# awslabs/crowd-coachable-recommendations

Hardware: AMD Instinct MI355X
Metric: queries/sec, exhaustive inner-product top-100 retrieval (NQ-shaped 2,681,468 x 768 bf16 corpus) (higher is better)
Workload: dtype bf16

## Files before the change

### crowd-coachable-recommendations_amd/ccrec_amd/_lib.py

```python
import ctypes
import os

_HERE = os.path.dirname(os.path.abspath(__file__))
LIB_PATH = os.path.join(os.path.dirname(_HERE), "lib", "libccr_hip.so")

CCR_OK = 0
CCR_ERR_INVALID, CCR_ERR_HIP, CCR_ERR_WORKSPACE, CCR_ERR_BLOCK_ID = -1, -2, -3, -4
DTYPE_F32, DTYPE_F16, DTYPE_BF16 = 0, 1, 2
SEARCH_DEFAULT, SEARCH_FORCE_DENSE, SEARCH_FORCE_FUSED, SEARCH_ASYNC = 0, 1, 2, 4
SCORES_CANONICAL, SCORES_MFMA = 0, 1

EXPORTS = [
    "ccr_last_error", "ccr_version", "ccr_pack_bf16", "ccr_pack_bf16_ex", "ccr_meanpool_pack_bf16", "ccr_meanpool_pack_bf16_ex", "ccr_index_create",
    "ccr_index_create_with_norms", "ccr_index_destroy",
    "ccr_index_rows", "ccr_index_dim", "ccr_search_workspace_bytes", "ccr_search", "ccr_search_last_stats",
    "ccr_merge_topk", "ccr_merge_topk_strided", "ccr_apply_block", "ccr_inbatch_ce_workspace_bytes", "ccr_inbatch_ce_fwd", "ccr_inbatch_ce_bwd", "ccr_inbatch_ce_bwd_dev", "ccr_rank_metrics",
    "ccr_search_finish", "ccr_scores", "ccr_search_blocked_workspace_bytes", "ccr_search_blocked",
    "ccr_search_sparse_prior_workspace_bytes", "ccr_search_sparse_prior", "ccr_colsum_bf16", "ccr_meanpool_bwd", "ccr_bm25_index_create", "ccr_bm25_index_destroy", "ccr_bm25_search_workspace_bytes",
    "ccr_bm25_search", "ccr_pack_bf16_padded", "ccr_shard_message_bytes", "ccr_search_shard", "ccr_shard_message_fill", "ccr_merge_shard_messages",
    "ccr_attention_bf16", "ccr_add_layernorm", "ccr_meanpool_pack_bf16_packed", "ccr_embed_layernorm", "ccr_gelu_bf16",
    "ccr_attention_half", "ccr_add_layernorm_half", "ccr_embed_layernorm_half", "ccr_gelu_half", "ccr_merge_short_lists",
    "ccr_bm25_search_workspace_bytes_k", "ccr_bm25_search_last_stats", "ccr_bm25_index_set_idf", "ccr_inbatch_pack3_bf16", "ccr_inbatch_ce_fwd_f32",
    "ccr_search_stream_wait_main_pass", "ccr_pool_ce_workspace_bytes", "ccr_pool_ce_fwd", "ccr_pool_ce_fwd_f32", "ccr_pool_ce_bwd_dev",
    "ccr_bpr_sample", "ccr_bpr_frozen_workspace_bytes", "ccr_bpr_frozen_fwd", "ccr_bpr_frozen_bwd_dev",
# ... 14 lines not shown
QSPLIT_VERSION = 105
THR_PHASES_VERSION = 106
OPTIM_VERSION = 107
ENCODER_PACKED_TRAIN_VERSION = 108
HALF_INDEX_VERSION = 109
AMP_OPTIM_VERSION = 110

SHARD_HEADER_BYTES = 32
SHARD_MAGIC = 0x4D524343


class ShardHeader(ctypes.Structure):
    _fields_ = [("magic", ctypes.c_uint32), ("n_flagged", ctypes.c_uint32), ("k_valid", ctypes.c_uint32),
                ("n_covered", ctypes.c_uint32), ("row_offset", ctypes.c_int64), ("n_rows", ctypes.c_int64)]


class SearchStats(ctypes.Structure):
    _fields_ = [("path", ctypes.c_int32), ("n_fallback", ctypes.c_int32), ("sample_tiles", ctypes.c_int32),
                ("ranges", ctypes.c_int32), ("cap", ctypes.c_int32), ("sublists", ctypes.c_int32),
                ("n_candidates", ctypes.c_int64), ("ms_sample", ctypes.c_float), ("ms_threshold", ctypes.c_float),
                ("ms_main", ctypes.c_float), ("ms_select", ctypes.c_float), ("ms_fallback", ctypes.c_float),
                ("ms_total", ctypes.c_float), ("n_retried", ctypes.c_int32), ("n_dense", ctypes.c_int32),
                ("main_launches", ctypes.c_int32), ("opt_rank", ctypes.c_int32), ("main_tile_queries", ctypes.c_int32),
                ("skipped_tiles", ctypes.c_int32)]


class AdamwSegment(ctypes.Structure):
    _fields_ = [("param", ctypes.c_void_p), ("grad", ctypes.c_void_p), ("exp_avg", ctypes.c_void_p), ("exp_avg_sq", ctypes.c_void_p),
                ("shadow", ctypes.c_void_p), ("n", ctypes.c_int64), ("decay", ctypes.c_float), ("step_size", ctypes.c_float),
                ("bc2_sqrt", ctypes.c_float), ("shadow_dtype", ctypes.c_int32)]


class AdamwControl(ctypes.Structure):
    _fields_ = [("coef", ctypes.c_float), ("skip", ctypes.c_int32), ("norm", ctypes.c_float), ("scale", ctypes.c_float),
                ("growth_tracker", ctypes.c_int32), ("skipped_total", ctypes.c_int32), ("reserved", ctypes.c_uint32 * 10)]


CONTROL_WORDS = {name: i for i, (name, _) in enumerate(AdamwControl._fields_[:6])}


class CcrError(RuntimeError):
    pass


_lib = None


# ... 140 lines not shown
```

### crowd-coachable-recommendations_amd/csrc/ccr_api.hip

```cpp
#include <stdarg.h>
#include <stdlib.h>
#include <string.h>

#include <math.h>

#include <algorithm>
#include <mutex>
#include <set>
#include <utility>
#include <vector>

#include "ccr_index.h"
#include "ccr_narrow.h"
#include "ccr_topk_device.h"

namespace ccr {

static thread_local char g_err[512] = "";
void set_error(const char *fmt, ...) {
    va_list ap;
    va_start(ap, fmt);
    vsnprintf(g_err, sizeof(g_err), fmt, ap);
    va_end(ap);
}
// ... 403 lines not shown
    return CCR_OK;
}


static int fused_stats(ccr_index *ix, uint32_t nflag, unsigned long long ncand) {
    const Plan &p = ix->plan;
    ccr_search_stats &st = ix->stats;
    float a = 0, b = 0;
    CCR_HIP_CHECK(hipEventElapsedTime(&st.ms_sample, ix->ev[EV_SAMPLE_BEGIN], ix->ev[EV_SAMPLE_END]));
    CCR_HIP_CHECK(hipEventElapsedTime(&a, ix->ev[EV_BEGIN], ix->ev[EV_SAMPLE_BEGIN]));
    CCR_HIP_CHECK(hipEventElapsedTime(&b, ix->ev[EV_SAMPLE_END], ix->ev[EV_MAIN_BEGIN]));
    st.ms_threshold = a + b;
    CCR_HIP_CHECK(hipEventElapsedTime(&st.ms_main, ix->ev[EV_MAIN_BEGIN], ix->ev[EV_MAIN_END]));
    CCR_HIP_CHECK(hipEventElapsedTime(&st.ms_select, ix->ev[EV_MAIN_END], ix->ev[EV_SELECT_END]));
    CCR_HIP_CHECK(hipEventElapsedTime(&st.ms_total, ix->ev[EV_BEGIN], ix->ev[EV_SELECT_END]));
    st.path = 1;
    st.n_fallback = (int32_t)nflag;
    st.sample_tiles = p.sample_tiles;
    st.ranges = p.narrow ? 1 : p.ranges;
    st.cap = p.narrow ? p.first_lay.cap[0] : p.cap;
    st.sublists = p.narrow ? p.first_sp : p.sublists;
    st.main_launches = 1 + (p.item_a ? 1 : 0) + (p.item_b ? 1 : 0);
    st.opt_rank = p.opt_rank;
    st.skipped_tiles = p.skip_sampled ? p.sample_tiles : 0;
    st.main_tile_queries = p.narrow ? 0 : p.tile_q;
    st.n_candidates = (int64_t)ncand;
    return CCR_OK;
}

static int recover_thresholds(const ccr_index *ix, const SearchWs &w, int nflag) {
    hipStream_t s = ix->pending.stream;
    ThresholdArgs t = threshold_args(ix, w);
    t.thr = w.thr_safe, t.cq = w.cq_safe;
    const int rc = launch_threshold(t, s);
    if (rc != CCR_OK) return rc;
    return launch_underfilled_to_retry(w.flag_list, 0, nflag, w.thr_safe, w.thr, s);
}

static int to_dense(const SearchWs &w, const uint32_t *list, int n, int &n_dense, hipStream_t s) {
    CCR_HIP_CHECK(hipMemcpyAsync(w.dense_list + n_dense, list, (size_t)n * 4, hipMemcpyDeviceToDevice, s));
    n_dense += n;
    return CCR_OK;
}

static int retry_group(ccr_index *ix, const SearchWs &w, const uint32_t *cur, int n_cur, int &n_dense) {
    const Plan &p = ix->plan;
// ... 189 lines not shown
        ix->have_events = true;
    }
    CCR_HIP_CHECK(hipEventRecord(ix->ev[EV_BEGIN], s));
    if (!p.fused) return search_dense(ix, w, Q_bf16, n_q, k, out_scores, out_ids, flags, s);
    ix->pending = {false, Q_bf16, n_q, k, out_scores, out_ids, (char *)workspace, s};

    CCR_HIP_CHECK(hipMemsetAsync(w.flag_count, 0, 64, s));
    if ((int64_t)p.ranges > p.tiles - (p.skip_sampled ? p.sample_tiles : 0)) CCR_HIP_CHECK(hipMemsetAsync(w.cnt, 0, (size_t)p.ranges * p.nq_pad * p.sublists * 4, s));
    int rc = launch_row_norms(Q_bf16, ix->dtype, n_q, ix->dim, w.qnorm, nullptr, nullptr, s);
    if (rc != CCR_OK) return rc;

    GemmArgs gs = gemm_args(ix, Q_bf16, n_q, p.nq_pad);
    gs.qgroups = p.qgroups;
    gs.n_vt = p.sample_tiles;
    gs.tile_stride = p.sample_stride;
    gs.ranges = p.sample_ranges;
    gs.gmax = w.gmax;
    CCR_HIP_CHECK(hipEventRecord(ix->ev[EV_SAMPLE_BEGIN], s));
    rc = launch_gemm(gs, ix->dtype, MAIN_32X32, EPI_GMAX, p.grid, s);
    if (rc != CCR_OK) return rc;
    CCR_HIP_CHECK(hipEventRecord(ix->ev[EV_SAMPLE_END], s));
    const bool skip_list = p.skip_sampled && ix->knobs.skip_list;
    ThresholdArgs t = threshold_args(ix, w);
    if (p.opt_rank) t.k = p.opt_rank;
    if (p.narrow) t.zero_cnt = w.cnt, t.zero_per_query = NARROW_SUBLISTS;
    if (skip_list) t.glist = w.glist, t.list_cap = skip_list_cap(p.opt_rank);
    rc = launch_threshold(t, s, &ix->thr_phases_used);
    if (rc != CCR_OK) return rc;

    CCR_HIP_CHECK(hipEventRecord(ix->ev[EV_MAIN_BEGIN], s));
    rc = p.narrow ? run_narrow_pass(ix, p, w, Q_bf16, n_q, s) : run_main_pass(ix, p, w, Q_bf16, n_q, s);
    if (rc != CCR_OK) return rc;
    CCR_HIP_CHECK(hipEventRecord(ix->ev[EV_MAIN_END], s));
    ix->main_pass_recorded = true;
    SelectArgs sel = select_args(ix, w);
    sel.ranges = p.first_nsub, sel.sp = p.first_sp, sel.lay = p.first_lay;
    sel.flag_count = w.flag_count, sel.flag_list = w.flag_list, sel.stat_cand = w.stat_cand;
    if (p.skip_sampled)
        sel.gmax = w.gmax, sel.sample_tiles = p.sample_tiles, sel.sample_stride = (int)p.sample_stride, sel.gmax_pitch = p.nq_pad;
    if (skip_list) sel.glist = w.glist, sel.list_cap = t.list_cap;
    rc = launch_select_rescore(sel, s);
    if (rc != CCR_OK) return rc;
    CCR_HIP_CHECK(hipEventRecord(ix->ev[EV_SELECT_END], s));

    if (!async) return search_complete(ix);
    if (flagged_out) CCR_HIP_CHECK(hipMemcpyAsync(flagged_out, w.flag_count, 4, hipMemcpyDeviceToDevice, s));
    CCR_HIP_CHECK(hipMemcpyAsync((void *)ix->host_flags, w.flag_count, 16, hipMemcpyDeviceToHost, s));
// ... 50 lines not shown
```

### crowd-coachable-recommendations_amd/csrc/ccr_index.h

```cpp
#pragma once
#include "ccr_common.h"
#include "ccr_plan.h"

namespace ccr {

enum MainKernel { MAIN_32X32, MAIN_16X16, MAIN_WIDE };
int launch_gemm(const GemmArgs &a, int dt, MainKernel kind, int epi, int grid, hipStream_t s);
int launch_shard_header(const ccr_shard_header &h, void *message, hipStream_t s);
int ensure_dynamic_lds(const void *kernel, size_t lds);
int launch_row_norms(const uint16_t *X, int dt, int64_t rows, int dim, float *norms, uint32_t *max_bits, uint32_t *tile_bits,
                     hipStream_t s);
int launch_tile_norms(const float *row_bounds, int64_t rows, uint32_t *tile_bits, uint32_t *max_bits, hipStream_t s);

struct ThresholdArgs {
    const float *gmax;
    int64_t n_groups, sample_stride;
    int n_q, nq_pad, dim;
    int k;
    const float *qnorm, *tile_norm;
    const uint32_t *dmax_bits;
    float *thr, *cq;
    uint32_t *zero_cnt = nullptr; int zero_per_query = 0;
    uint32_t *glist = nullptr; int list_cap = 0;
    int phases = 0;
};
int launch_threshold(const ThresholdArgs &a, hipStream_t s, int *phases_used = nullptr);

struct ThresholdUpdateArgs {
    const uint2 *cand;
    const uint32_t *cnt;
    CandLayout lay;
    int sp;
    int n_q, nq_pad, k, nsub;
    const float *cq, *tile_norm;
    float *thr;
    int nsub_part = 0, part_blocks = 0, prev_nsub = 0, prev_part = 0, prev_blocks = 0;
    int qb_per = 1;
    uint32_t *top = nullptr;
    bool top_in = false, top_out = false;
    int tile_q = TILE_Q;
};
// ... 83 lines not shown
```

### crowd-coachable-recommendations_amd/csrc/ccr_plan.h

```cpp
#pragma once
#include "ccr_common.h"
#include "ccr_narrow.h"

namespace ccr {

struct Knobs {
    int qgroups;
    int progressive;
    int max_phases;
    int mfma16;
    int sample_div;
    int ranges;
    int optimistic;
    int opt_rank;
    int max_lists;
    int narrow;
    int narrow_grid;
    int skip_sampled;
    int skip_list;
    int qsplit;
    int wide;
    int thr_phases;
    int narrow_groups;
};
struct KnobDef {
    const char *env;
    int Knobs::*field;
    int dflt;
};
inline constexpr KnobDef KNOB_DEFS[] = {
    {"CCR_QGROUPS", &Knobs::qgroups, 0},           {"CCR_PROGRESSIVE", &Knobs::progressive, 1},   {"CCR_PHASES", &Knobs::max_phases, 3},
    {"CCR_MFMA16", &Knobs::mfma16, -1},            {"CCR_SAMPLE_DIV", &Knobs::sample_div, 0},     {"CCR_RANGES", &Knobs::ranges, 0},
    {"CCR_OPTIMISTIC", &Knobs::optimistic, -1},    {"CCR_OPT_RANK", &Knobs::opt_rank, 0},         {"CCR_MAX_LISTS", &Knobs::max_lists, 0},
    {"CCR_NARROW", &Knobs::narrow, -1},            {"CCR_NARROW_GRID", &Knobs::narrow_grid, 0},   {"CCR_SKIP_SAMPLED", &Knobs::skip_sampled, -1},
    {"CCR_SKIP_LIST", &Knobs::skip_list, 1},       {"CCR_QSPLIT", &Knobs::qsplit, -1},            {"CCR_WIDE", &Knobs::wide, -1},
    {"CCR_THR_PHASES", &Knobs::thr_phases, 0},     {"CCR_NARROW_GROUPS", &Knobs::narrow_groups, NARROW_MAX_GROUPS},
};
static_assert(sizeof(KNOB_DEFS) / sizeof(KNOB_DEFS[0]) * sizeof(int) == sizeof(Knobs), "a row for every knob");
inline Knobs default_knobs() {
    Knobs kn;
    for (const KnobDef &d : KNOB_DEFS) kn.*d.field = d.dflt;
    return kn;
}
Knobs read_knobs();

struct Plan {
    int fused;
    int nq_pad;
    int qblocks;
    int tile_q;
    int main_qblocks;
    int main_qgroups;
    int main_qsplit;
    int64_t tiles;
    int64_t full_tiles;
    int sample_tiles;
    int64_t sample_stride;
    int sample_ranges;
    int ranges;
    int item_a;
    int item_b;
    int opt_rank;
    int skip_sampled;
    int qgroups;
    int cap;
    CandLayout cand;
    int grid;
    int rescore_cap;
    int rescore_regular;
    int select_compact;
    int mfma16;
    int sublists;
    int narrow;
    int narrow_groups;
    int first_nsub;
    int first_sp;
    CandLayout first_lay;
    int64_t cand_recs;
    size_t total;
    int64_t dense_rows_per_chunk;
};

constexpr int FALLBACK_ROWS = 16;

Plan make_plan(int64_t n_rows, int dim, int n_q, int k, int flags, int num_cu, const Knobs &kn);

inline int64_t round_up(int64_t v, int64_t m) { return (v + m - 1) / m * m; }
int pick_qgroups(int qblocks, int dim, const Knobs &kn, int tile_q = TILE_Q);
CandLayout one_segment(int cap);

struct Bump {
    size_t off;
    size_t take(size_t bytes) { const size_t o = off; off = (off + bytes + 255) / 256 * 256; return o; }
};

struct SearchWs {
    float *qnorm, *thr, *cq, *gmax;
    uint32_t *cnt;
    uint2 *cand;
    uint32_t *flag_count, *flag_list;
    unsigned long long *stat_cand;
    uint32_t *top;
    float *thr_safe, *cq_safe, *dense;
    uint32_t *glist;
// ... 10 lines not shown
```

### crowd-coachable-recommendations_amd/csrc/ccr_plan.hip

```cpp
#include <stdlib.h>
#include <string.h>

#include <math.h>

#include <algorithm>
#include <vector>

#include "ccr_index.h"
#include "ccr_topk_device.h"

namespace ccr {

Knobs read_knobs() {
    Knobs kn = default_knobs();
    for (const KnobDef &d : KNOB_DEFS)
        if (const char *e = getenv(d.env)) kn.*d.field = atoi(e);
    return kn;
}

constexpr double L2_RESIDENT_BYTES = 3.2 * 1048576.0, L2_MOSTLY_BYTES = 5.5 * 1048576.0;
constexpr double WIDE_TILE_COST = 1.37;
constexpr double MODEL_QUERIES = 3584.0;

static double tile_cost(const Plan &p) { return p.tile_q == WIDE_Q ? WIDE_TILE_COST : 1.0; }
static double query_scale(const Plan &p) { return (double)p.nq_pad / MODEL_QUERIES; }

static double gamma_upper(double r) { return 1.25 * (r + 4.75 * sqrt(r) + 8.0) / r; }

static double estimated_pass(int rank, double fs, int k) { return std::max((double)rank / fs, (double)k); }
static double sample_fraction(const Plan &p) { return 1.0 / ((double)p.tiles / (double)p.sample_tiles); }
static double estimated_pass_upper(const Plan &p, int k) {
    return gamma_upper((double)p.opt_rank) * estimated_pass(p.opt_rank, sample_fraction(p), k);
}
static double conservative_pass(const Plan &p, int k) { return (double)k * ((double)p.tiles / (double)p.sample_tiles) * 1.3 + 64.0; }

int pick_qgroups(int qblocks, int dim, const Knobs &kn, int tile_q) {
    {
        const int v = kn.qgroups;
        if ((v == 1 || v == 2 || v == 4 || v == 8) && qblocks % v == 0) return v;
    }
    const size_t block_bytes = (size_t)tile_q * dim * 2;
    int best = 1;
    for (int gq = 1; gq <= NUM_XCD; gq *= 2) {
        if (qblocks % gq) continue;
        best = gq;
        if ((size_t)(qblocks / gq) * block_bytes <= (size_t)3 << 20) break;
    }
    return best;
}

static int footprint_class(double bytes) { return bytes <= L2_RESIDENT_BYTES ? 0 : (bytes <= L2_MOSTLY_BYTES ? 1 : 2); }

static int pick_qsplit(int qblocks, int equal_groups, int dim, int tile_q, const Knobs &kn) {
    if (kn.qsplit == 0) return 0;
    const int v = kn.qgroups;
// ... 32 lines not shown
        }
    }
    return best_r;
}

constexpr size_t DENSE_SCRATCH_TARGET = (size_t)1 << 30;

struct MainPassChoice {
    int64_t sample, ranges;
    int item_a, item_b;
    int opt_rank;
    int skip;
};

static bool may_skip_sampled(const Plan &p, int64_t sample, const Knobs &kn) {
    if (kn.skip_sampled == 0 || p.narrow || sample < 1) return false;
    const int64_t stride = std::max<int64_t>(1, p.full_tiles / sample);
    return stride >= 2 && (sample - 1) * stride < p.full_tiles && sample < p.tiles;
}

static int optimistic_rank(int k, int64_t sample, int64_t tiles, const Knobs &kn, bool skip = false) {
    if (kn.opt_rank > 0) return kn.opt_rank;
    const double need = (double)k * (double)sample / (double)(skip ? tiles - sample : tiles);
    int r = 40;
    for (; r < 1 << 20; ++r) {
        const double a = 1.0 / (9.0 * r), t = 1.0 - a - 5.2 * sqrt(a);
        if (t > 0.0 && (double)r * t * t * t >= need) break;
    }
    return r;
}

static void range_window(const Plan &p, const Knobs &kn, int64_t &r_hi, int64_t &target) {
    int64_t max_lists = p.rescore_cap > 512 ? 2048 : 1024;
    if ((max_lists / p.sublists) * p.main_qblocks < p.grid) max_lists = 2048;
    if (kn.max_lists >= 64 && kn.max_lists < max_lists) max_lists = kn.max_lists;
    r_hi = std::min<int64_t>(max_lists / p.sublists, round_up(std::max<int64_t>(1, p.tiles / 8), NUM_XCD));
    target = std::min<int64_t>(r_hi, round_up(std::max<int64_t>(NUM_XCD, (int64_t)p.grid * 6 / p.main_qblocks), NUM_XCD));
}

static double sample_cost(const Plan &p, int64_t smp) {
    return (double)((smp * p.qblocks + p.grid - 1) / p.grid) + 0.015 * (double)smp * std::max(1.0, query_scale(p));
}

struct Best {
    double cost;
    MainPassChoice choice;
    void offer(double c, const MainPassChoice &ch) {
        if (c < cost) cost = c, choice = ch;
    }
};

static void price_range_count(const Plan &p, int k, const Knobs &kn, int64_t smp, int64_t R, int64_t target, bool reprice_skipped, Best &best) {
    const int nrc = NUM_XCD / p.main_qgroups, qb_per = p.main_qblocks / p.main_qgroups, per_x = p.grid / NUM_XCD;
    const double qscale = query_scale(p);
    const double select_per_range = 0.1 * qscale, hit_w = 0.014 * qscale, phase_w = 3.0;
    const double fs = (double)smp / (double)p.tiles;
    auto survivors = [&](double fa, double fb) -> double {
        if (fa <= 0.0) return (double)k / fs;
        if (fb <= 0.0) return (double)k * (fa / fs + (1.0 - fa) / fa);
        return (double)k * (fa / fs + fb / fa + (1.0 - fa - fb) / (fa + fb));
    };
    const int64_t items = R / nrc * qb_per;
    const double item_cost = ((double)((p.tiles + R - 1) / R) + 0.15) * tile_cost(p);
    auto rounds = [&](int64_t n) { return (double)((n + per_x - 1) / per_x); };
    const double common = sample_cost(p, smp) + select_per_range * (double)R + 1e-3 * std::abs((double)(R - target));
    const double single = rounds(items) * item_cost + hit_w * survivors(0.0, 0.0) + common;
    if (kn.optimistic != 1 && !reprice_skipped) best.offer(single, {smp, R, 0, 0, 0, 0});
    if (kn.optimistic != 0 && smp * GROUPS_PER_TILE >= 4 * 40) {
        const bool skip = reprice_skipped && may_skip_sampled(p, smp, kn);
        const int rank = optimistic_rank(k, smp, p.tiles, kn, skip);
        if ((int64_t)rank * 4 <= smp * GROUPS_PER_TILE) {
            const double opt_item = skip ? ((double)((p.tiles - smp + R - 1) / R) + 0.15) * tile_cost(p) : item_cost;
            const double opt = rounds(items) * opt_item + hit_w * estimated_pass(rank, fs, k) + common - (kn.optimistic == 1 ? 1e9 : 0.0);
            best.offer(opt, {smp, R, 0, 0, rank, skip ? 1 : 0});
        }
    }
    if (reprice_skipped || kn.progressive == 0 || p.narrow || !(items > per_x && (double)p.tiles / (double)R >= 8.0)) return;
    const double fa = (double)per_x / (double)items;
    best.offer((1.0 + rounds(items - per_x)) * item_cost + phase_w + hit_w * survivors(fa, 0.0) + common, {smp, R, per_x, 0, 0, 0});
    if (kn.max_phases < 3) return;
    for (int ph = 1; ph <= 3; ++ph) {
        const int64_t ib = (int64_t)per_x * (1 + ph);
        if (ib >= items) break;
        const double fb = (double)ph * per_x / (double)items;
        best.offer((1.0 + ph + rounds(items - ib)) * item_cost + 2.0 * phase_w + hit_w * survivors(fa, fb) + common, {smp, R, per_x, (int)ib, 0, 0});
    }
}

static MainPassChoice choose_main_pass(const Plan &p, int k, const std::vector<int64_t> &samples, const Knobs &kn, bool reprice_skipped = false) {
    int64_t r_hi, target;
    range_window(p, kn, r_hi, target);
// ... 72 lines not shown
    p.narrow = narrow ? nqt : 0;
    p.narrow_groups = narrow ? ngroups : 1;
}

static void choose_tile(const Search &s, Plan &p) {
    const Knobs &kn = s.kn;
    const int n_q = s.n_q, dim = s.dim;
    if (!p.narrow && p.mfma16 && dim % 32 == 0 && kn.wide != 0) {
        static const double per_flop_of_class[3] = {0.95, 0.97, 1.04};
        const int wb = (n_q + WIDE_Q - 1) / WIDE_Q;
        const double per_xcd = (double)(wb / pick_qgroups(wb, dim, kn, WIDE_Q)) * WIDE_Q * dim * 2.0;
        const double per_flop = per_flop_of_class[footprint_class(per_xcd)];
        if (kn.wide == 1 || (double)wb * WIDE_Q * per_flop < (double)p.qblocks * TILE_Q) {
            p.tile_q = WIDE_Q;
            p.main_qblocks = wb;
            p.nq_pad = (int)round_up(std::max<int64_t>(n_q, (int64_t)wb * WIDE_Q), TILE_Q);
            p.qblocks = p.nq_pad / TILE_Q;
            p.qgroups = pick_qgroups(p.qblocks, dim, kn);
        }
    }
    p.main_qgroups = pick_qgroups(p.main_qblocks, dim, kn, p.tile_q);
}

static void choose_launches(const Search &s, Plan &p, const std::vector<int64_t> &samples) {
    const Knobs &kn = s.kn;
    MainPassChoice choice = choose_main_pass(p, s.k, samples, kn);
    if (choice.opt_rank > 0 && may_skip_sampled(p, choice.sample, kn)) {
        const MainPassChoice skipped = choose_main_pass(p, s.k, {choice.sample}, kn, true);
        if (skipped.skip) choice = skipped;
    }
    p.sample_tiles = (int)choice.sample;
    p.sample_stride = std::max<int64_t>(1, p.full_tiles / choice.sample);
    p.sample_ranges = best_sample_ranges(choice.sample, p.qblocks, p.qgroups, p.grid);
    p.ranges = (int)choice.ranges;
    p.item_a = choice.item_a;
    p.item_b = choice.item_b;
    p.opt_rank = choice.opt_rank;
    p.skip_sampled = (p.opt_rank > 0 && !p.narrow) ? choice.skip : 0;
    p.main_qsplit = (!p.narrow && p.item_a == 0 && p.item_b == 0) ? pick_qsplit(p.main_qblocks, p.main_qgroups, s.dim, p.tile_q, kn) : 0;
}

static void price_skip_sampled(const Search &s, Plan &p) {
    if (!p.skip_sampled) return;
    const int k = s.k;
    const double join_rows = 256.0 * (double)p.sample_tiles * (1.0 - pow(1.0 - std::min(1.0, (double)k / (double)s.n_rows), 16.0));
    const double need = (double)k + (double)(k / 4) + 1.5 * join_rows + TILE_DOCS + 16;
    const double saved = 0.5 * (double)p.sample_tiles * p.main_qblocks * tile_cost(p) / (double)p.grid;
    const bool pays = 0.065 * join_rows * query_scale(p) < saved;
    if (need > 8192.0 || (s.kn.skip_sampled < 0 && !pays))
        p.skip_sampled = 0;
    else
        p.rescore_cap = std::min(8192, std::max(p.rescore_cap, pow2_ceil((int)need)));
}

CandLayout one_segment(int cap) {
    CandLayout L;
    memset(&L, 0, sizeof(L));
    L.nseg = 1;
    L.seg_end[0] = L.seg_end[1] = L.seg_end[2] = INT32_MAX;
    L.cap[0] = L.cap[1] = L.cap[2] = cap;
    return L;
}

static void plan_candidates(const Search &s, Plan &p) {
    const int k = s.k;
    const int64_t R = p.ranges;
    const int nrc_p = NUM_XCD / p.main_qgroups, qb_per_p = p.main_qblocks / p.main_qgroups;
    auto ranges_to = [&](int item) { return item ? std::min<int64_t>(R, (int64_t)nrc_p * ((item + qb_per_p - 1) / qb_per_p)) : 0; };
    const int64_t RA = ranges_to(p.item_a), RB = ranges_to(p.item_b);
    const double fs = sample_fraction(p), nlists = (double)R * p.sublists;
    const double xk = gamma_upper((double)k);
    const int64_t tile_rows = TILE_DOCS / p.sublists;
    auto cap_for = [&](double g) -> int {
        const double mean = p.opt_rank ? estimated_pass_upper(p, k) / nlists : xk * (double)k / (g * nlists);
// ... 139 lines not shown
```

### crowd-coachable-recommendations_amd/csrc/ccr_threshold.hip

```cpp
#include <algorithm>

#include "ccr_gemm_common.h"
#include "ccr_index.h"
#include "ccr_topk_device.h"

namespace ccr {

template <int ET>
__global__ __launch_bounds__(256) void row_norms_kernel(const uint16_t *__restrict__ X, int64_t rows, int dim,
                                                            float *__restrict__ norms, uint32_t *__restrict__ max_bits,
                                                            uint32_t *__restrict__ tile_bits) {
    const int lane = threadIdx.x & 63;
    const int64_t wave = ((int64_t)blockIdx.x * blockDim.x + threadIdx.x) >> 6;
    const int64_t nwaves = ((int64_t)gridDim.x * blockDim.x) >> 6;
    const int chunk = tile_bits ? 64 : 1;
    uint32_t wbits = 0u;
    for (int64_t r0 = wave * chunk; r0 < rows; r0 += nwaves * chunk) {
        uint32_t cbits = 0u;
        const int64_t r1 = r0 + chunk < rows ? r0 + chunk : rows;
        for (int64_t r = r0; r < r1; ++r) {
            const uint16_t *x = X + r * dim;
            float s = 0.f;
            for (int c = lane * 8; c < dim; c += 64 * 8) {
                const uint4 v = *reinterpret_cast<const uint4 *>(x + c);
// ... 59 lines not shown
}

int launch_row_norms(const uint16_t *X, int dt, int64_t rows, int dim, float *norms, uint32_t *max_bits, uint32_t *tile_bits,
                     hipStream_t s) {
    if (rows <= 0) return CCR_OK;
    int64_t blocks = tile_bits ? (rows + 255) / 256 : (rows + 3) / 4;
    if (blocks > 2048) blocks = 2048;
    return dispatch_half(dt, [&](auto et) {
        hipLaunchKernelGGL(row_norms_kernel<decltype(et)::value>, dim3((unsigned)blocks), dim3(256), 0, s, X, rows, dim, norms, max_bits, tile_bits);
        CCR_LAUNCH_CHECK();
        return CCR_OK;
    });
}

int launch_tile_norms(const float *row_bounds, int64_t rows, uint32_t *tile_bits, uint32_t *max_bits, hipStream_t s) {
    if (rows <= 0) return CCR_OK;
    const int64_t tiles = (rows + TILE_DOCS - 1) / TILE_DOCS;
    hipLaunchKernelGGL(tile_norms_kernel, dim3((unsigned)tiles), dim3(256), 0, s, row_bounds, rows, tile_bits);
    hipLaunchKernelGGL(max_tile_norm_kernel, dim3(1), dim3(1024), 0, s, tile_bits, tiles, max_bits);
    CCR_LAUNCH_CHECK();
    return CCR_OK;
}

constexpr int THR_WIDE_QUERIES = 16;
constexpr int THR_WIDE_MIN_BATCHES = 2;

template <bool LIST, int PH, int QB>
__global__ __launch_bounds__(QB * PH) void threshold_kernel(const float *__restrict__ gmax, int64_t n_groups, int n_q, int nq_pad,
                                                           int k, const float *__restrict__ qnorm,
                                                           const uint32_t *__restrict__ dmax_bits, float gamma,
                                                           const float *__restrict__ tile_norm, int64_t sample_stride,
                                                           float *__restrict__ thr, float *__restrict__ cq,
                                                           uint32_t *__restrict__ glist, int list_cap) {
    constexpr int THREADS = QB * PH;
    constexpr int PICK = QB * 16;
    static_assert(THREADS >= PICK && PICK % 64 == 0 && (QB & (QB - 1)) == 0, "threshold_kernel: shape");
    __shared__ uint32_t s_hist[QB][256];
    __shared__ uint32_t s_prefix[QB], s_remaining[QB], s_nlist[QB];
    const int tid = threadIdx.x;
    const int ql = tid & (QB - 1), ph = tid / QB;
    const int q = blockIdx.x * QB + ql;
    if (tid < QB) {
        s_prefix[tid] = 0;
        s_remaining[tid] = (uint32_t)k;
        s_nlist[tid] = 0;
    }
    uint32_t *const my_list = LIST ? glist + (int64_t)q * (list_cap + 1) : nullptr;

    const float dmax = __uint_as_float(*dmax_bits);
    const float c = (q < n_q) ? ((dmax < INFINITY) ? gamma * (qnorm[q] * 1.001f) * 1.001f : __builtin_nanf("")) : 0.f;
    auto tile_of = [&](int64_t g) { return tile_norm[(g / GROUPS_PER_TILE) * sample_stride]; };
    auto emit = [&](int64_t g, float v, float tn, uint32_t prefix) {
        if (f32_orderable(fmaf(c, tn, v)) >= prefix) {
            const uint32_t p = atomicAdd(&s_nlist[ql], 1u);
            if (p < (uint32_t)list_cap) my_list[1 + p] = (uint32_t)g;
        }
    };
    uint32_t mask = 0;
    for (int shift = 24; shift >= 0; shift -= 8) {
        const bool listing = LIST && shift == 0;
        for (int b = tid; b < QB * 256; b += THREADS) (&s_hist[0][0])[b] = 0;
        CCR_WAIT_LGKM0();
        __syncthreads();
        const uint32_t prefix = s_prefix[ql];
        int64_t i = ph;
        for (; i + 15 * PH < n_groups; i += 16 * PH) {
            float v[16], tn[16];
#pragma unroll
            for (int j = 0; j < 16; ++j) {
                v[j] = gmax[(i + PH * j) * nq_pad + q];
                tn[j] = tile_of(i + PH * j);
            }
#pragma unroll
            for (int j = 0; j < 16; ++j) {
                const uint32_t o = f32_orderable(fmaf(-c, tn[j], v[j]));
                if ((o & mask) == prefix) atomicAdd(&s_hist[ql][(o >> shift) & 255u], 1u);
                if (listing) emit(i + PH * j, v[j], tn[j], prefix);
            }
        }
        for (; i < n_groups; i += PH) {
            const float v = gmax[i * nq_pad + q], tn = tile_of(i);
            const uint32_t o = f32_orderable(fmaf(-c, tn, v));
            if ((o & mask) == prefix) atomicAdd(&s_hist[ql][(o >> shift) & 255u], 1u);
            if (listing) emit(i, v, tn, prefix);
        }
        CCR_WAIT_LGKM0();
        __syncthreads();
        const bool picker = tid < PICK;
        const int qi = (tid >> 4) & (QB - 1), part = tid & 15;
        uint32_t remaining = 0, own = 0, incl = 0, above = 0, total = 0;
        uint32_t hb[16];
        if (picker) {
            remaining = s_remaining[qi];
#pragma unroll
            for (int j = 0; j < 16; ++j) {
                hb[j] = s_hist[qi][16 * part + j];
                own += hb[j];
            }
            incl = own;
#pragma unroll
            for (int off = 1; off < 16; off <<= 1) {
                const uint32_t t = __shfl_down(incl, off, 16);
                if (part + off < 16) incl += t;
            }
            above = incl - own;
            total = __shfl(incl, 0, 16);
        }
// ... 12 lines not shown
                    cum += hb[j];
                }
                s_prefix[qi] |= (uint32_t)d << shift;
                s_remaining[qi] = remaining - cum;
            } else if (part == 0 && total < remaining) {
                s_remaining[qi] = remaining - (total - hb[0]);
            }
        }
        mask |= 0xffu << shift;
        CCR_WAIT_LGKM0();
        __syncthreads();
    }
    if (tid < QB) {
        const int qq = blockIdx.x * QB + tid;
        if (qq < n_q) {
            const float tau = orderable_to_f32(s_prefix[tid]);
            cq[qq] = c;
            thr[qq] = (c < INFINITY) ? tau : __builtin_nanf("");
        }
        if (LIST) my_list[0] = s_nlist[tid];
    }
}

__global__ __launch_bounds__(256) void threshold_small_kernel(const float *__restrict__ gmax, int n_groups, int nq_pad, int k,
                                                             const float *__restrict__ qnorm, const uint32_t *__restrict__ dmax_bits,
                                                             float gamma, const float *__restrict__ tile_norm, int64_t sample_stride,
                                                             float *__restrict__ thr, float *__restrict__ cq, uint32_t *__restrict__ zero_cnt,
                                                             int zero_per_query, uint32_t *__restrict__ glist, int list_cap) {
    extern __shared__ __attribute__((aligned(16))) uint32_t s_low[];
    __shared__ uint32_t s_hist[256];
    __shared__ uint32_t s_ctl[4];
    __shared__ uint32_t s_nlist;
    const int tid = threadIdx.x, q = blockIdx.x;
    const float dmax = __uint_as_float(*dmax_bits);
    const float c = (dmax < INFINITY) ? gamma * (qnorm[q] * 1.001f) * 1.001f : __builtin_nanf("");
    for (int g = tid; g < n_groups; g += 256)
        s_low[g] = f32_orderable(fmaf(-c, tile_norm[(int64_t)(g / GROUPS_PER_TILE) * sample_stride], gmax[(int64_t)g * nq_pad + q]));
    if (zero_cnt && tid < zero_per_query) zero_cnt[q * zero_per_query + tid] = 0u;
    __syncthreads();
    uint32_t kth = 0;
    int need_eq = 0;
    block_radix_select<true>(
        [&](int64_t i, bool &skip) -> uint32_t {
            (void)skip;
            return s_low[i];
        },
        n_groups, k, s_hist, s_ctl, kth, need_eq);
    if (tid == 0) {
        cq[q] = c;
        thr[q] = (c < INFINITY) ? orderable_to_f32(kth) : __builtin_nanf("");
    }
    if (glist) {
        uint32_t *const my_list = glist + (int64_t)q * (list_cap + 1);
        if (tid == 0) s_nlist = 0u;
        __syncthreads();
        for (int g = tid; g < n_groups; g += 256) {
            const float up = fmaf(c, tile_norm[(int64_t)(g / GROUPS_PER_TILE) * sample_stride], gmax[(int64_t)g * nq_pad + q]);
            if (f32_orderable(up) >= kth) {
                const uint32_t p = atomicAdd(&s_nlist, 1u);
                if (p < (uint32_t)list_cap) my_list[1 + p] = (uint32_t)g;
            }
        }
        __syncthreads();
        if (tid == 0) my_list[0] = s_nlist;
    }
}

int launch_threshold(const ThresholdArgs &a, hipStream_t s, int *phases_used) {
    if (phases_used) *phases_used = 0;
    if (a.n_q <= 128 && a.n_groups >= a.k && a.n_groups <= 16384 && a.zero_per_query <= 256) {
        if (a.n_groups * 4 > 32 * 1024) {
            const int rc = ensure_dynamic_lds(reinterpret_cast<const void *>(&threshold_small_kernel), 72 * 1024);
            if (rc != CCR_OK) return rc;
        }
        hipLaunchKernelGGL(threshold_small_kernel, dim3(a.n_q), dim3(256), (size_t)a.n_groups * 4, s, a.gmax, (int)a.n_groups, a.nq_pad, a.k,
                           a.qnorm, a.dmax_bits, mfma_gamma(a.dim), a.tile_norm, a.sample_stride, a.thr, a.cq, a.zero_cnt, a.zero_per_query,
                           a.glist, a.list_cap);
        CCR_LAUNCH_CHECK();
        return CCR_OK;
    }
    if (a.zero_cnt) CCR_HIP_CHECK(hipMemsetAsync(a.zero_cnt, 0, (size_t)a.n_q * a.zero_per_query * 4, s));
    const bool wide = a.phases == 64 || (a.phases != 16 && a.n_groups >= (int64_t)THR_WIDE_MIN_BATCHES * 16 * 64);
    if (phases_used) *phases_used = wide ? 64 : 16;
    const auto kernel = wide ? (a.glist ? threshold_kernel<true, 64, THR_WIDE_QUERIES> : threshold_kernel<false, 64, THR_WIDE_QUERIES>)
                             : (a.glist ? threshold_kernel<true, 16, 16> : threshold_kernel<false, 16, 16>);
    const int qb = wide ? THR_WIDE_QUERIES : 16, ph = wide ? 64 : 16;
    hipLaunchKernelGGL(kernel, dim3(a.nq_pad / qb), dim3(qb * ph), 0, s, a.gmax, a.n_groups, a.n_q, a.nq_pad, a.k, a.qnorm, a.dmax_bits,
                       mfma_gamma(a.dim), a.tile_norm, a.sample_stride, a.thr, a.cq, a.glist, a.list_cap);
    CCR_LAUNCH_CHECK();
    return CCR_OK;
}

__global__ __launch_bounds__(256) void threshold_update_kernel(const uint2 *__restrict__ cand, const uint32_t *__restrict__ cnt,
                                                              int nsub_full, int nsub_part, int part_blocks, int prev_full,
                                                              int prev_part, int prev_blocks, int qb_per, int sp, int nq_pad,
                                                              const CandLayout lay, int k, int compact,
                                                              const float *__restrict__ cq, const float *__restrict__ tile_norm,
                                                              uint32_t *__restrict__ top, int top_in, int top_out,
                                                              float *__restrict__ thr, int tile_q) {
    extern __shared__ __attribute__((aligned(16))) uint32_t s_val[];
    __shared__ uint32_t s_hist[256];
    __shared__ uint32_t s_ctl[4];
    __shared__ uint32_t s_cnt[2048];
    __shared__ uint32_t s_total, s_maxc, s_fill, s_eq;
    const int tid = threadIdx.x;
    const int q = blockIdx.x;
    const int qpos = (q / tile_q) % qb_per;
    const int nsub = qpos < part_blocks ? nsub_part : nsub_full;
    uint32_t *top_n = top;
    uint32_t *top_v = top ? top + nq_pad + (int64_t)q * k : nullptr;
// ... 114 lines not shown
```

### include/ccr_retrieval.h

```cpp
#ifndef CCR_RETRIEVAL_H
#define CCR_RETRIEVAL_H

#include <stddef.h>
#include <stdint.h>

#ifdef __cplusplus
extern "C" {
#endif

#define CCR_OK 0
#define CCR_ERR_INVALID (-1)
#define CCR_ERR_HIP (-2)
#define CCR_ERR_WORKSPACE (-3)
#define CCR_ERR_BLOCK_ID (-4)

#define CCR_DTYPE_F32 0
#define CCR_DTYPE_F16 1
#define CCR_DTYPE_BF16 2

#define CCR_SEARCH_DEFAULT 0
#define CCR_SEARCH_FORCE_DENSE 1
#define CCR_SEARCH_FORCE_FUSED 2
#define CCR_SEARCH_ASYNC 4

// ... 2 lines not shown

typedef struct ccr_index ccr_index;

typedef struct ccr_search_stats {
    int32_t path;
    int32_t n_fallback;
    int32_t sample_tiles;
    int32_t ranges;
    int32_t cap;
    int32_t sublists;
    int64_t n_candidates;
    float ms_sample;
    float ms_threshold;
    float ms_main;
    float ms_select;
    float ms_fallback;
    float ms_total;
    int32_t n_retried;
    int32_t n_dense;
    int32_t main_launches;
    int32_t opt_rank;
    int32_t main_tile_queries;
    int32_t skipped_tiles;
} ccr_search_stats;

const char *ccr_last_error(void);
int ccr_version(void);

int ccr_pack_bf16(const float *src, uint16_t *dst, float *norms, int64_t rows, int dim, int normalize, void *stream);
int ccr_pack_bf16_ex(const float *src, uint16_t *dst, float *norms, float *row_norm_bounds, int64_t rows, int dim, int normalize,
                     void *stream);

int ccr_pack_bf16_padded(const float *src, int64_t rows, int src_dim, uint16_t *dst, int dst_dim, float *norms,
                         float *row_norm_bounds, int normalize, void *stream);

int ccr_meanpool_pack_bf16(const void *hidden, int hidden_dtype, const int64_t *mask, uint16_t *dst_bf16,
                           float *dst_f32, int B, int L, int dim, int normalize, void *stream);
int ccr_meanpool_pack_bf16_ex(const void *hidden, int hidden_dtype, const int64_t *mask, uint16_t *dst_bf16,
                              float *dst_f32, const int64_t *dst_rows, float *row_norm_bounds, int B, int L, int dim,
                              int normalize, void *stream);

int ccr_meanpool_pack_bf16_packed(const void *hidden, int hidden_dtype, const int32_t *seq_start, const int32_t *seq_len,
                                  uint16_t *dst_bf16, float *dst_f32, const int64_t *dst_rows, float *row_norm_bounds, int n_seq,
                                  int dim, int normalize, void *stream);

int ccr_pack_half_ex(const float *src, uint16_t *dst, float *norms, float *row_norm_bounds, int64_t rows, int dim, int normalize,
// ... 228 lines not shown
```

Baseline: 258,200.

## Cap per-tile group contributions in threshold rank to allow lower optimistic rank

The threshold kernels now count only the top tile_cap group maxima in each sampled tile when building the rank histogram. This lets the planner pick a lower optimistic rank (down to OPT_RANK_MIN) when sampled tiles are skipped. The intent is a tighter pruning threshold, so fewer candidates survive the main pass and selection. The cost is extra per-tile sorting work in the threshold kernel, plus a higher risk of underfilled queries and retries.

```diff
diff --git a/crowd-coachable-recommendations_amd/ccrec_amd/_lib.py b/crowd-coachable-recommendations_amd/ccrec_amd/_lib.py
--- a/crowd-coachable-recommendations_amd/ccrec_amd/_lib.py
+++ b/crowd-coachable-recommendations_amd/ccrec_amd/_lib.py
@@ -60,7 +60,7 @@
                 ("ms_main", ctypes.c_float), ("ms_select", ctypes.c_float), ("ms_fallback", ctypes.c_float),
                 ("ms_total", ctypes.c_float), ("n_retried", ctypes.c_int32), ("n_dense", ctypes.c_int32),
                 ("main_launches", ctypes.c_int32), ("opt_rank", ctypes.c_int32), ("main_tile_queries", ctypes.c_int32),
-                ("skipped_tiles", ctypes.c_int32)]
+                ("skipped_tiles", ctypes.c_int32), ("tile_cap", ctypes.c_int32)]
 
 
 class AdamwSegment(ctypes.Structure):
diff --git a/crowd-coachable-recommendations_amd/csrc/ccr_api.hip b/crowd-coachable-recommendations_amd/csrc/ccr_api.hip
--- a/crowd-coachable-recommendations_amd/csrc/ccr_api.hip
+++ b/crowd-coachable-recommendations_amd/csrc/ccr_api.hip
@@ -449,6 +449,7 @@
     st.sublists = p.narrow ? p.first_sp : p.sublists;
     st.main_launches = 1 + (p.item_a ? 1 : 0) + (p.item_b ? 1 : 0);
     st.opt_rank = p.opt_rank;
+    st.tile_cap = p.opt_rank ? p.tile_cap : 0;
     st.skipped_tiles = p.skip_sampled ? p.sample_tiles : 0;
     st.main_tile_queries = p.narrow ? 0 : p.tile_q;
     st.n_candidates = (int64_t)ncand;
@@ -684,7 +685,7 @@
     CCR_HIP_CHECK(hipEventRecord(ix->ev[EV_SAMPLE_END], s));
     const bool skip_list = p.skip_sampled && ix->knobs.skip_list;
     ThresholdArgs t = threshold_args(ix, w);
-    if (p.opt_rank) t.k = p.opt_rank;
+    if (p.opt_rank) t.k = p.opt_rank, t.tile_cap = p.tile_cap;
     if (p.narrow) t.zero_cnt = w.cnt, t.zero_per_query = NARROW_SUBLISTS;
     if (skip_list) t.glist = w.glist, t.list_cap = skip_list_cap(p.opt_rank);
     rc = launch_threshold(t, s, &ix->thr_phases_used);
diff --git a/crowd-coachable-recommendations_amd/csrc/ccr_index.h b/crowd-coachable-recommendations_amd/csrc/ccr_index.h
--- a/crowd-coachable-recommendations_amd/csrc/ccr_index.h
+++ b/crowd-coachable-recommendations_amd/csrc/ccr_index.h
@@ -17,6 +17,7 @@
     int64_t n_groups, sample_stride;
     int n_q, nq_pad, dim;
     int k;
+    int tile_cap = GROUPS_PER_TILE;
     const float *qnorm, *tile_norm;
     const uint32_t *dmax_bits;
     float *thr, *cq;
diff --git a/crowd-coachable-recommendations_amd/csrc/ccr_plan.h b/crowd-coachable-recommendations_amd/csrc/ccr_plan.h
--- a/crowd-coachable-recommendations_amd/csrc/ccr_plan.h
+++ b/crowd-coachable-recommendations_amd/csrc/ccr_plan.h
@@ -22,6 +22,7 @@
     int wide;
     int thr_phases;
     int narrow_groups;
+    int tile_cap;
 };
 struct KnobDef {
     const char *env;
@@ -35,6 +36,7 @@
     {"CCR_NARROW", &Knobs::narrow, -1},            {"CCR_NARROW_GRID", &Knobs::narrow_grid, 0},   {"CCR_SKIP_SAMPLED", &Knobs::skip_sampled, -1},
     {"CCR_SKIP_LIST", &Knobs::skip_list, 1},       {"CCR_QSPLIT", &Knobs::qsplit, -1},            {"CCR_WIDE", &Knobs::wide, -1},
     {"CCR_THR_PHASES", &Knobs::thr_phases, 0},     {"CCR_NARROW_GROUPS", &Knobs::narrow_groups, NARROW_MAX_GROUPS},
+    {"CCR_TILE_CAP", &Knobs::tile_cap, 0},
 };
 static_assert(sizeof(KNOB_DEFS) / sizeof(KNOB_DEFS[0]) * sizeof(int) == sizeof(Knobs), "a row for every knob");
 inline Knobs default_knobs() {
@@ -61,6 +63,8 @@
     int item_a;
     int item_b;
     int opt_rank;
+    int tile_cap;
+    int cap_rank;
     int skip_sampled;
     int qgroups;
     int cap;
@@ -80,6 +84,10 @@
     size_t total;
     int64_t dense_rows_per_chunk;
 };
+
+constexpr int TILE_CAP_MIN = 4, TILE_CAP_TILES = 5;
+constexpr int OPT_RANK_MIN = TILE_CAP_MIN * (TILE_CAP_TILES - 1) + 1;
+constexpr int OPT_RANK_FLOOR = 40, REDUCED_RANK_MIN_TILES = 40;
 
 constexpr int FALLBACK_ROWS = 16;
 
diff --git a/crowd-coachable-recommendations_amd/csrc/ccr_plan.hip b/crowd-coachable-recommendations_amd/csrc/ccr_plan.hip
--- a/crowd-coachable-recommendations_amd/csrc/ccr_plan.hip
+++ b/crowd-coachable-recommendations_amd/csrc/ccr_plan.hip
@@ -30,7 +30,7 @@
 static double estimated_pass(int rank, double fs, int k) { return std::max((double)rank / fs, (double)k); }
 static double sample_fraction(const Plan &p) { return 1.0 / ((double)p.tiles / (double)p.sample_tiles); }
 static double estimated_pass_upper(const Plan &p, int k) {
-    return gamma_upper((double)p.opt_rank) * estimated_pass(p.opt_rank, sample_fraction(p), k);
+    return gamma_upper((double)p.cap_rank) * estimated_pass(p.cap_rank, sample_fraction(p), k);
 }
 static double conservative_pass(const Plan &p, int k) { return (double)k * ((double)p.tiles / (double)p.sample_tiles) * 1.3 + 64.0; }
 
@@ -109,12 +109,20 @@
 static int optimistic_rank(int k, int64_t sample, int64_t tiles, const Knobs &kn, bool skip = false) {
     if (kn.opt_rank > 0) return kn.opt_rank;
     const double need = (double)k * (double)sample / (double)(skip ? tiles - sample : tiles);
-    int r = 40;
+    int r = (skip && sample >= REDUCED_RANK_MIN_TILES) ? OPT_RANK_MIN : OPT_RANK_FLOOR;
     for (; r < 1 << 20; ++r) {
         const double a = 1.0 / (9.0 * r), t = 1.0 - a - 5.2 * sqrt(a);
         if (t > 0.0 && (double)r * t * t * t >= need) break;
     }
     return r;
+}
+
+static int tile_cap_for(int rank, int64_t sample, const Knobs &kn) {
+    int cap = (rank + TILE_CAP_TILES - 1) / TILE_CAP_TILES;
+    cap = std::min(GROUPS_PER_TILE, std::max(TILE_CAP_MIN, cap));
+    if (kn.tile_cap >= 1 && kn.tile_cap <= GROUPS_PER_TILE) cap = kn.tile_cap;
+    const int64_t fill = ((int64_t)rank + sample - 1) / std::max<int64_t>(1, sample);
+    return (int)std::min<int64_t>(GROUPS_PER_TILE, std::max<int64_t>(cap, fill));
 }
 
 static void range_window(const Plan &p, const Knobs &kn, int64_t &r_hi, int64_t &target) {
@@ -153,7 +161,7 @@
     const double common = sample_cost(p, smp) + select_per_range * (double)R + 1e-3 * std::abs((double)(R - target));
     const double single = rounds(items) * item_cost + hit_w * survivors(0.0, 0.0) + common;
     if (kn.optimistic != 1 && !reprice_skipped) best.offer(single, {smp, R, 0, 0, 0, 0});
-    if (kn.optimistic != 0 && smp * GROUPS_PER_TILE >= 4 * 40) {
+    if (kn.optimistic != 0 && smp * GROUPS_PER_TILE >= 160) {
         const bool skip = reprice_skipped && may_skip_sampled(p, smp, kn);
         const int rank = optimistic_rank(k, smp, p.tiles, kn, skip);
         if ((int64_t)rank * 4 <= smp * GROUPS_PER_TILE) {
@@ -272,6 +280,11 @@
     p.main_qgroups = pick_qgroups(p.main_qblocks, dim, kn, p.tile_q);
 }
 
+static void set_rank_dependents(Plan &p, const Knobs &kn) {
+    p.tile_cap = p.opt_rank > 0 ? tile_cap_for(p.opt_rank, p.sample_tiles, kn) : GROUPS_PER_TILE;
+    p.cap_rank = (kn.opt_rank > 0 || p.opt_rank == 0) ? p.opt_rank : std::max(p.opt_rank, OPT_RANK_FLOOR);
+}
+
 static void choose_launches(const Search &s, Plan &p, const std::vector<int64_t> &samples) {
     const Knobs &kn = s.kn;
     MainPassChoice choice = choose_main_pass(p, s.k, samples, kn);
@@ -286,6 +299,7 @@
     p.item_a = choice.item_a;
     p.item_b = choice.item_b;
     p.opt_rank = choice.opt_rank;
+    set_rank_dependents(p, kn);
     p.skip_sampled = (p.opt_rank > 0 && !p.narrow) ? choice.skip : 0;
     p.main_qsplit = (!p.narrow && p.item_a == 0 && p.item_b == 0) ? pick_qsplit(p.main_qblocks, p.main_qgroups, s.dim, p.tile_q, kn) : 0;
 }
@@ -297,9 +311,11 @@
     const double need = (double)k + (double)(k / 4) + 1.5 * join_rows + TILE_DOCS + 16;
     const double saved = 0.5 * (double)p.sample_tiles * p.main_qblocks * tile_cost(p) / (double)p.grid;
     const bool pays = 0.065 * join_rows * query_scale(p) < saved;
-    if (need > 8192.0 || (s.kn.skip_sampled < 0 && !pays))
+    if (need > 8192.0 || (s.kn.skip_sampled < 0 && !pays)) {
         p.skip_sampled = 0;
-    else
+        p.opt_rank = std::max(p.opt_rank, optimistic_rank(k, p.sample_tiles, p.tiles, s.kn, false));
+        set_rank_dependents(p, s.kn);
+    } else
         p.rescore_cap = std::min(8192, std::max(p.rescore_cap, pow2_ceil((int)need)));
 }
 
diff --git a/crowd-coachable-recommendations_amd/csrc/ccr_threshold.hip b/crowd-coachable-recommendations_amd/csrc/ccr_threshold.hip
--- a/crowd-coachable-recommendations_amd/csrc/ccr_threshold.hip
+++ b/crowd-coachable-recommendations_amd/csrc/ccr_threshold.hip
@@ -105,12 +105,30 @@
     return CCR_OK;
 }
 
+__device__ __forceinline__ uint32_t tile_top_mask(const uint32_t (&o)[GROUPS_PER_TILE], int cap) {
+    int before[GROUPS_PER_TILE];
+#pragma unroll
+    for (int j = 0; j < GROUPS_PER_TILE; ++j) before[j] = GROUPS_PER_TILE - 1 - j;
+#pragma unroll
+    for (int i = 0; i < GROUPS_PER_TILE; ++i)
+#pragma unroll
+        for (int j = i + 1; j < GROUPS_PER_TILE; ++j) {
+            const int first = o[i] >= o[j] ? 1 : 0;
+            before[j] += first;
+            before[i] -= first;
+        }
+    uint32_t in = 0u;
+#pragma unroll
+    for (int j = 0; j < GROUPS_PER_TILE; ++j) in |= (before[j] < cap ? 1u : 0u) << j;
+    return in;
+}
+
 constexpr int THR_WIDE_QUERIES = 16;
 constexpr int THR_WIDE_MIN_BATCHES = 2;
 
 template <bool LIST, int PH, int QB>
 __global__ __launch_bounds__(QB * PH) void threshold_kernel(const float *__restrict__ gmax, int64_t n_groups, int n_q, int nq_pad,
-                                                           int k, const float *__restrict__ qnorm,
+                                                           int k, int tile_cap, const float *__restrict__ qnorm,
                                                            const uint32_t *__restrict__ dmax_bits, float gamma,
                                                            const float *__restrict__ tile_norm, int64_t sample_stride,
                                                            float *__restrict__ thr, float *__restrict__ cq,
@@ -132,7 +150,8 @@
 
     const float dmax = __uint_as_float(*dmax_bits);
     const float c = (q < n_q) ? ((dmax < INFINITY) ? gamma * (qnorm[q] * 1.001f) * 1.001f : __builtin_nanf("")) : 0.f;
-    auto tile_of = [&](int64_t g) { return tile_norm[(g / GROUPS_PER_TILE) * sample_stride]; };
+    auto tile_of = [&](int64_t t) { return tile_norm[t * sample_stride]; };
+    const int64_t n_tiles = n_groups / GROUPS_PER_TILE;
     auto emit = [&](int64_t g, float v, float tn, uint32_t prefix) {
         if (f32_orderable(fmaf(c, tn, v)) >= prefix) {
             const uint32_t p = atomicAdd(&s_nlist[ql], 1u);
@@ -146,26 +165,23 @@
         CCR_WAIT_LGKM0();
         __syncthreads();
         const uint32_t prefix = s_prefix[ql];
-        int64_t i = ph;
-        for (; i + 15 * PH < n_groups; i += 16 * PH) {
-            float v[16], tn[16];
-#pragma unroll
-            for (int j = 0; j < 16; ++j) {
-                v[j] = gmax[(i + PH * j) * nq_pad + q];
-                tn[j] = tile_of(i + PH * j);
-            }
-#pragma unroll
-            for (int j = 0; j < 16; ++j) {
-                const uint32_t o = f32_orderable(fmaf(-c, tn[j], v[j]));
-                if ((o & mask) == prefix) atomicAdd(&s_hist[ql][(o >> shift) & 255u], 1u);
-                if (listing) emit(i + PH * j, v[j], tn[j], prefix);
-            }
-        }
-        for (; i < n_groups; i += PH) {
-            const float v = gmax[i * nq_pad + q], tn = tile_of(i);
-            const uint32_t o = f32_orderable(fmaf(-c, tn, v));
-            if ((o & mask) == prefix) atomicAdd(&s_hist[ql][(o >> shift) & 255u], 1u);
-            if (listing) emit(i, v, tn, prefix);
+        for (int64_t t = ph; t < n_tiles; t += PH) {
+            const int64_t g0 = t * GROUPS_PER_TILE;
+            float v[GROUPS_PER_TILE];
+            uint32_t o[GROUPS_PER_TILE];
+#pragma unroll
+            for (int j = 0; j < GROUPS_PER_TILE; ++j) v[j] = gmax[(g0 + j) * nq_pad + q];
+            const float tn = tile_of(t);
+            if (listing) {
+#pragma unroll
+                for (int j = 0; j < GROUPS_PER_TILE; ++j) emit(g0 + j, v[j], tn, prefix);
+            }
+#pragma unroll
+            for (int j = 0; j < GROUPS_PER_TILE; ++j) o[j] = f32_orderable(fmaf(-c, tn, v[j]));
+            const uint32_t in = tile_cap < GROUPS_PER_TILE ? tile_top_mask(o, tile_cap) : 0xffffu;
+#pragma unroll
+            for (int j = 0; j < GROUPS_PER_TILE; ++j)
+                if (((in >> j) & 1u) && (o[j] & mask) == prefix) atomicAdd(&s_hist[ql][(o[j] >> shift) & 255u], 1u);
         }
         CCR_WAIT_LGKM0();
         __syncthreads();
@@ -224,7 +240,7 @@
     }
 }
 
-__global__ __launch_bounds__(256) void threshold_small_kernel(const float *__restrict__ gmax, int n_groups, int nq_pad, int k,
+__global__ __launch_bounds__(256) void threshold_small_kernel(const float *__restrict__ gmax, int n_groups, int nq_pad, int k, int tile_cap,
                                                              const float *__restrict__ qnorm, const uint32_t *__restrict__ dmax_bits,
                                                              float gamma, const float *__restrict__ tile_norm, int64_t sample_stride,
                                                              float *__restrict__ thr, float *__restrict__ cq, uint32_t *__restrict__ zero_cnt,
@@ -236,8 +252,20 @@
     const int tid = threadIdx.x, q = blockIdx.x;
     const float dmax = __uint_as_float(*dmax_bits);
     const float c = (dmax < INFINITY) ? gamma * (qnorm[q] * 1.001f) * 1.001f : __builtin_nanf("");
-    for (int g = tid; g < n_groups; g += 256)
-        s_low[g] = f32_orderable(fmaf(-c, tile_norm[(int64_t)(g / GROUPS_PER_TILE) * sample_stride], gmax[(int64_t)g * nq_pad + q]));
+    if (tile_cap < GROUPS_PER_TILE) {
+        for (int t = tid; t < n_groups / GROUPS_PER_TILE; t += 256) {
+            const float tn = tile_norm[(int64_t)t * sample_stride];
+            uint32_t o[GROUPS_PER_TILE];
+#pragma unroll
+            for (int j = 0; j < GROUPS_PER_TILE; ++j) o[j] = f32_orderable(fmaf(-c, tn, gmax[(int64_t)(t * GROUPS_PER_TILE + j) * nq_pad + q]));
+            const uint32_t in = tile_top_mask(o, tile_cap);
+#pragma unroll
+            for (int j = 0; j < GROUPS_PER_TILE; ++j) s_low[t * GROUPS_PER_TILE + j] = ((in >> j) & 1u) ? o[j] : 0u;
+        }
+    } else {
+        for (int g = tid; g < n_groups; g += 256)
+            s_low[g] = f32_orderable(fmaf(-c, tile_norm[(int64_t)(g / GROUPS_PER_TILE) * sample_stride], gmax[(int64_t)g * nq_pad + q]));
+    }
     if (zero_cnt && tid < zero_per_query) zero_cnt[q * zero_per_query + tid] = 0u;
     __syncthreads();
     uint32_t kth = 0;
@@ -270,13 +298,21 @@
 
 int launch_threshold(const ThresholdArgs &a, hipStream_t s, int *phases_used) {
     if (phases_used) *phases_used = 0;
+    if (a.n_groups % GROUPS_PER_TILE || a.tile_cap < 1) {
+        set_error("threshold: %lld groups are not whole tiles, or tile cap %d", (long long)a.n_groups, a.tile_cap);
+        return CCR_ERR_INVALID;
+    }
+    if (a.tile_cap < GROUPS_PER_TILE && (int64_t)a.tile_cap * (a.n_groups / GROUPS_PER_TILE) < a.k) {
+        set_error("threshold: rank %d above the %d x %lld groups the tile cap leaves", a.k, a.tile_cap, (long long)(a.n_groups / GROUPS_PER_TILE));
+        return CCR_ERR_INVALID;
+    }
     if (a.n_q <= 128 && a.n_groups >= a.k && a.n_groups <= 16384 && a.zero_per_query <= 256) {
         if (a.n_groups * 4 > 32 * 1024) {
             const int rc = ensure_dynamic_lds(reinterpret_cast<const void *>(&threshold_small_kernel), 72 * 1024);
             if (rc != CCR_OK) return rc;
         }
         hipLaunchKernelGGL(threshold_small_kernel, dim3(a.n_q), dim3(256), (size_t)a.n_groups * 4, s, a.gmax, (int)a.n_groups, a.nq_pad, a.k,
-                           a.qnorm, a.dmax_bits, mfma_gamma(a.dim), a.tile_norm, a.sample_stride, a.thr, a.cq, a.zero_cnt, a.zero_per_query,
+                           a.tile_cap, a.qnorm, a.dmax_bits, mfma_gamma(a.dim), a.tile_norm, a.sample_stride, a.thr, a.cq, a.zero_cnt, a.zero_per_query,
                            a.glist, a.list_cap);
         CCR_LAUNCH_CHECK();
         return CCR_OK;
@@ -287,7 +323,7 @@
     const auto kernel = wide ? (a.glist ? threshold_kernel<true, 64, THR_WIDE_QUERIES> : threshold_kernel<false, 64, THR_WIDE_QUERIES>)
                              : (a.glist ? threshold_kernel<true, 16, 16> : threshold_kernel<false, 16, 16>);
     const int qb = wide ? THR_WIDE_QUERIES : 16, ph = wide ? 64 : 16;
-    hipLaunchKernelGGL(kernel, dim3(a.nq_pad / qb), dim3(qb * ph), 0, s, a.gmax, a.n_groups, a.n_q, a.nq_pad, a.k, a.qnorm, a.dmax_bits,
+    hipLaunchKernelGGL(kernel, dim3(a.nq_pad / qb), dim3(qb * ph), 0, s, a.gmax, a.n_groups, a.n_q, a.nq_pad, a.k, a.tile_cap, a.qnorm, a.dmax_bits,
                        mfma_gamma(a.dim), a.tile_norm, a.sample_stride, a.thr, a.cq, a.glist, a.list_cap);
     CCR_LAUNCH_CHECK();
     return CCR_OK;
diff --git a/include/ccr_retrieval.h b/include/ccr_retrieval.h
--- a/include/ccr_retrieval.h
+++ b/include/ccr_retrieval.h
@@ -48,6 +48,7 @@
     int32_t opt_rank;
     int32_t main_tile_queries;
     int32_t skipped_tiles;
+    int32_t tile_cap;
 } ccr_search_stats;
 
 const char *ccr_last_error(void);
```

After: 264,400, median of 6. 1.02x the previous value.
